# NikNazarov/TorchPIV

Measured on AMD Instinct MI355X. Metric: image-pairs/sec at 4 MP, wind=64 ov=32 2-pass CWS; % HBM roofline, higher is better.
Workload: dtype u32 exact sums + f64 / f32

## Files before the change

torchpiv_amd/csrc/xcorr_exact.hip:

```cpp
#include <hip/hip_runtime.h>
#include <stdint.h>
#include <stdlib.h>

#include "piv_kernels.h"
#include "xcorr_tile.hpp"

namespace tpiv {

namespace {

template <int W>
struct XGeo {
    static constexpr int NDW = W / 4;
    static constexpr int XP = 2 * NDW + 1;
    static constexpr int GROUP = W < 64 ? W : 64;
    static constexpr int WPW = 64 / GROUP;
    static constexpr int PARTS = W / GROUP;
    static constexpr int WAVES = W == 128 || W == 64 ? 2 : 4;
    static constexpr int WINS = WAVES * WPW / PARTS;
    static constexpr int KD = W * W;
    static constexpr bool COOP = W >= 32;
    static constexpr int P16 = W / 16;
    static constexpr int LW = GROUP * PARTS;
    static constexpr int AP = NDW + 4;
    static_assert(!COOP || (W * AP <= W * XP && (LW * P16) == W * P16), "the hand-over tile lives in the parked rows' memory");
};
constexpr int XCELLS = 5 + EXACT_MAX_SECOND + EXACT_MAX_MIN;

#if defined(__HIP_DEVICE_COMPILE__)
template <int OFF>
__device__ __forceinline__ uint32_t lds_rd32(unsigned addr) {
    uint32_t v;
    asm volatile("ds_read_b32 %0, %1 offset:%2" : "=v"(v) : "v"(addr), "n"(OFF) : "memory");
    return v;
}
__device__ __forceinline__ void lds_landed() { asm volatile("s_waitcnt lgkmcnt(0)" ::: "memory"); }
__device__ __forceinline__ void lds_tie(uint32_t& v) { asm volatile("" : "+v"(v)); }
#else
template <int OFF>
__host__ __device__ inline uint32_t lds_rd32(unsigned) { return 0u; }
__host__ __device__ inline void lds_landed() {}
__host__ __device__ inline void lds_tie(uint32_t&) {}
#endif
template <int N>
__device__ __forceinline__ void read_span(const uint32_t* src, uint32_t (&w)[N]) {
    const unsigned addr = (unsigned)(uintptr_t)src;
    static_for<0, N>([&](auto ic) TPIV_LAMBDA_INLINE { w[decltype(ic)::value] = lds_rd32<4 * decltype(ic)::value>(addr); });
    lds_landed();
    static_for<0, N>([&](auto ic) TPIV_LAMBDA_INLINE { lds_tie(w[decltype(ic)::value]); });
}

__device__ __forceinline__ void list_append(const PassParams& p, bool want, long long it) {
    const unsigned long long mk = __ballot(want);
    if (mk == 0ull) return;
    const int lane = (int)__builtin_amdgcn_mbcnt_hi(~0u, __builtin_amdgcn_mbcnt_lo(~0u, 0u));
    const int leader = (int)__builtin_ctzll(mk);
    unsigned base = 0u;
    if (lane == leader) base = atomicAdd(p.fb_count, (unsigned)__popcll(mk));
    base = (unsigned)__builtin_amdgcn_readlane((int)base, leader);
    if (want) p.fb_list[base + (unsigned)__popcll(mk & ((1ull << lane) - 1ull))] = (int)it;
}

__device__ __forceinline__ void decide_and_store(const PassParams& p, const uint4& rec, int r0, bool go, bool writer, bool have,
                                                 int m, unsigned S, unsigned sa, unsigned sb, double kd, double* out, long long it) {
    auto hi16 = [](unsigned v) TPIV_LAMBDA_INLINE { return (int)(short)(v >> 16); };
    auto umin = [](unsigned x, unsigned y) TPIV_LAMBDA_INLINE { return x < y ? x : y; };
    auto umax = [](unsigned x, unsigned y) TPIV_LAMBDA_INLINE { return x > y ? x : y; };
    auto uadd = [](unsigned x, unsigned y) TPIV_LAMBDA_INLINE { return x + y; };
    constexpr int S0 = 5, N0 = 5 + EXACT_MAX_SECOND;
    S = r0 < XCELLS ? S : 0u;
    const unsigned s_min = grp_reduce<16>((have && r0 >= N0 && r0 < XCELLS) ? S : 0xffffffffu, umin);
    const unsigned s_low = grp_reduce<16>((have && r0 < XCELLS) ? S : 0xffffffffu, umin);
    const unsigned s_top = grp_reduce<16>((have && r0 < N0) ? S : 0u, umax);
    const unsigned s_m = grp_reduce<16>(r0 == 0 ? S : 0u, umax);
    const unsigned s_second = grp_reduce<16>((have && r0 >= S0 && r0 < N0) ? S : 0u, umax);
    const unsigned n_second = grp_reduce<16>((have && r0 >= S0 && r0 < N0) ? 1u : 0u, uadd);
    const bool min_overflow = hi16(rec.w) == -2;
    const bool redo = s_top > s_m || s_low < s_min || s_min == 0xffffffffu || sa == 0u || sb == 0u ||
                      (min_overflow && s_min != 0u);
    list_append(p, go && redo && r0 == 0 && writer, it);
    const double scale = (kd * kd) / ((double)sa * (double)sb);
    const unsigned mine = r0 == 5 ? s_second : S;
    double v = __fma_rn((double)(mine - s_min), scale, 1e-7);
    v = (r0 == 5 && n_second == 0u) ? 0.0 : v;
    v = r0 == 6 ? (double)m : v;
    v = r0 == 7 ? 0.0 : v;
    if (go && !redo && r0 < 8 && writer) out[r0] = v;
}

template <int W>
__global__ __launch_bounds__(64 * XGeo<W>::WAVES) void xcorr_exact_refine_kernel(PassParams p) {
    using G = XGeo<W>;
    constexpr int NDW = G::NDW, XP = G::XP, KD = G::KD;
    __shared__ __attribute__((aligned(16))) uint32_t parked[G::WINS][W * XP];
    __shared__ unsigned joined[2][16];
    const int wave = __builtin_amdgcn_readfirstlane((int)(threadIdx.x >> 6));
    const int lane = (int)(threadIdx.x & 63);
    const int g = lane / G::GROUP, r0 = lane % G::GROUP;
    const int part = G::PARTS == 2 ? wave : 0;
    const int row = r0 + 64 * part;
    const int wslot = G::PARTS == 2 ? 0 : wave * G::WPW + g;
    uint32_t* const rows_b = parked[wslot];
    const int N = p.n_rows * p.n_cols;
    const long long total = (long long)p.batch * N;
    const int xcd = blockIdx.x & 7, slot = blockIdx.x >> 3;
    const long long chunk = (total + 7) / 8;
    const long long in_chunk = (long long)slot * G::WINS + wslot;
    const long long it_raw = (long long)xcd * chunk + in_chunk;
    const bool valid = in_chunk < chunk && it_raw < total;
    const long long it = valid ? it_raw : 0;

    const unsigned itu = (unsigned)it;
    const int pair = (int)(itu / (unsigned)N), win = (int)(itu - (unsigned)pair * (unsigned)N);
    const int st = p.ws - p.ov;
    const size_t off0 = (size_t)pair * p.H * p.W + (size_t)((win / p.n_cols) * st) * p.W + (size_t)(win % p.n_cols) * st;
    uint32_t a[NDW], b[NDW];
    uint32_t ca[G::COOP ? G::P16 : 1][4], cb[G::COOP ? G::P16 : 1][4];
    const int tw = r0 + 64 * part;
    if constexpr (G::COOP) {
#pragma unroll
        for (int k = 0; k < G::P16; ++k) {
            const int ci = tw + G::LW * k, j = ci / G::P16, pt = ci % G::P16;
            const size_t o_ = off0 + (size_t)j * p.W + 16 * pt;
            load_dwords<4>(p.A + o_, ca[k]);
            load_dwords<4>(p.B + o_, cb[k]);
        }
    } else {
        const size_t off = off0 + (size_t)row * p.W;
        load_dwords<NDW>(p.A + off, a);
        load_dwords<NDW>(p.B + off, b);
    }
    const uint4 rec = p.cand[it];
    auto lo16 = [](unsigned v) TPIV_LAMBDA_INLINE { return (int)(short)(v & 0xffffu); };
    auto hi16 = [](unsigned v) TPIV_LAMBDA_INLINE { return (int)(short)(v >> 16); };
    const int m = valid ? lo16(rec.x) : -3;
    double* const out = reinterpret_cast<double*>(p.peak_raw) + (size_t)it * 8;
    const bool writer = part == 0;
    list_append(p, m == -1 && r0 == 0 && writer, it);
    if (m == -2 && r0 < 8 && writer) out[r0] = r0 == 6 ? 0.0 : 1.0;
    const bool go = m >= 0;
    if (__ballot(go) == 0ull) return;
    bool nb_fast = false;
    if constexpr (G::COOP) {
        const bool regular = (m & (W - 1)) >= 1 && (m & (W - 1)) <= W - 2 && m + 1 < KD - 1 && m - 1 > 0 && m + W < KD - 1 &&
                             m - W > 0;
        nb_fast = __ballot(go && !regular) == 0ull;
    }

    int q = -1;
    if (go) {
        int left = m + 1, right = m - 1, top = m + W, bot = m - W;
        if (left >= KD - 1) left = m;
        if (right <= 0) right = m;
        if (top >= KD - 1) top = m;
        if (bot <= 0) bot = m;
        q = r0 == 0 ? m : q;
        q = r0 == 1 ? left : q;
        q = r0 == 2 ? right : q;
        q = r0 == 3 ? top : q;
        q = r0 == 4 ? bot : q;
        q = r0 == 5 ? hi16(rec.x) : q;
        q = r0 == 6 ? lo16(rec.y) : q;
        q = r0 == 7 ? hi16(rec.y) : q;
        q = r0 == 8 ? lo16(rec.z) : q;
        q = r0 == 9 ? hi16(rec.z) : q;
        q = r0 == 10 ? lo16(rec.w) : q;
        q = r0 == 11 ? hi16(rec.w) : q;
    }

    unsigned P[16];
#pragma unroll
    for (int k = 0; k < 16; ++k) P[k] = 0u;
    auto lds_sync = [&]() TPIV_LAMBDA_INLINE {
        if constexpr (G::PARTS == 2) __syncthreads();
        else wave_sync();
    };
    uint32_t au[NDW], ad[NDW];
    if constexpr (G::COOP) {
        uint4* const ta = reinterpret_cast<uint4*>(rows_b);
#pragma unroll
        for (int k = 0; k < G::P16; ++k) {
            const int ci = tw + G::LW * k, j = ci / G::P16, pt = ci % G::P16;
            ta[j * (G::AP / 4) + pt] = make_uint4(ca[k][0], ca[k][1], ca[k][2], ca[k][3]);
        }
        lds_sync();
#pragma unroll
        for (int k = 0; k < NDW / 4; ++k) {
            const uint4 t = ta[row * (G::AP / 4) + k];
            a[4 * k] = t.x, a[4 * k + 1] = t.y, a[4 * k + 2] = t.z, a[4 * k + 3] = t.w;
        }
        if (nb_fast) {
            const int ru = (row - 1) & (W - 1), rd = (row + 1) & (W - 1);
#pragma unroll
            for (int k = 0; k < NDW / 4; ++k) {
                const uint4 t = ta[ru * (G::AP / 4) + k], s = ta[rd * (G::AP / 4) + k];
                au[4 * k] = t.x, au[4 * k + 1] = t.y, au[4 * k + 2] = t.z, au[4 * k + 3] = t.w;
                ad[4 * k] = s.x, ad[4 * k + 1] = s.y, ad[4 * k + 2] = s.z, ad[4 * k + 3] = s.w;
            }
        }
        lds_sync();
#pragma unroll
        for (int k = 0; k < G::P16; ++k) {
            const int ci = tw + G::LW * k, j = ci / G::P16, pt = ci % G::P16;
#pragma unroll
            for (int c = 0; c < 4; ++c) {
                P[13] = __builtin_amdgcn_sad_u8(cb[k][c], 0u, P[13]);
                rows_b[j * XP + 4 * pt + c] = cb[k][c];
                rows_b[j * XP + NDW + 4 * pt + c] = cb[k][c];
            }
        }
#pragma unroll
        for (int i = 0; i < NDW; ++i) P[12] = __builtin_amdgcn_sad_u8(a[i], 0u, P[12]);
    } else {
#pragma unroll
        for (int i = 0; i < NDW; ++i) {
            P[12] = __builtin_amdgcn_sad_u8(a[i], 0u, P[12]);
            P[13] = __builtin_amdgcn_sad_u8(b[i], 0u, P[13]);
            rows_b[row * XP + i] = b[i];
            rows_b[row * XP + NDW + i] = b[i];
        }
    }
    lds_sync();

    if constexpr (G::COOP) {
        if (nb_fast) {
            const int mm = go ? m : KD / 2 + W / 2;
            const int dy = mm / W - W / 2, s = (mm % W - W / 2 - 1) & (W - 1);
            const int brow = (row + dy) & (W - 1);
            uint32_t w[NDW + 2];
            read_span<NDW + 2>(rows_b + brow * XP + (s >> 2), w);
            w[NDW + 1] = s == W - 1 ? w[1] : w[NDW + 1];
            uint32_t u[NDW + 1];
#pragma unroll
            for (int i = 0; i <= NDW; ++i) u[i] = __builtin_amdgcn_alignbyte(w[i + 1], w[i], (unsigned)(s & 3));
            unsigned s_m = 0u, s_l = 0u, s_r = 0u, s_t = 0u, s_b = 0u;
#pragma unroll
            for (int i = 0; i < NDW; ++i) {
                const uint32_t c = __builtin_amdgcn_alignbyte(u[i + 1], u[i], 1u);
                s_r = __builtin_amdgcn_udot4(a[i], u[i], s_r, false);
                s_m = __builtin_amdgcn_udot4(a[i], c, s_m, false);
                s_l = __builtin_amdgcn_udot4(a[i], __builtin_amdgcn_alignbyte(u[i + 1], u[i], 2u), s_l, false);
                s_t = __builtin_amdgcn_udot4(au[i], c, s_t, false);
                s_b = __builtin_amdgcn_udot4(ad[i], c, s_b, false);
            }
            P[0] = go ? s_m : 0u, P[1] = go ? s_l : 0u, P[2] = go ? s_r : 0u, P[3] = go ? s_t : 0u, P[4] = go ? s_b : 0u;
        }
    }
    static_for<0, XCELLS>([&](auto cc) TPIV_LAMBDA_INLINE {
        constexpr int c = decltype(cc)::value;
        if (c < 5 && nb_fast) return;
        int qc = __builtin_amdgcn_readlane(q, c);
        bool any = qc >= 0;
        static_for<1, G::WPW>([&](auto wc) TPIV_LAMBDA_INLINE {
            constexpr int k = decltype(wc)::value;
            const int qk = __builtin_amdgcn_readlane(q, k * G::GROUP + c);
            any = any || qk >= 0;
            qc = g == k ? qk : qc;
        });
        if (any) {
            const bool on = qc >= 0;
            const int qq = on ? qc : 0;
            const int dy = qq / W - W / 2, dx = qq % W - W / 2;
            const int brow = (row + dy) & (W - 1), bx = dx & (W - 1);
            const uint32_t* src = rows_b + brow * XP + (bx >> 2);
            const unsigned sh = (unsigned)(bx & 3);
            uint32_t w[NDW + 1];
            read_span<NDW + 1>(src, w);
            unsigned acc = 0;
#pragma unroll
            for (int i = 0; i < NDW; ++i) acc = __builtin_amdgcn_udot4(a[i], __builtin_amdgcn_alignbyte(w[i + 1], w[i], sh), acc, false);
            P[c] = on ? acc : 0u;
        }
    });
    unsigned T[4];
    {
        const bool odd = lane & 1, hi = lane & 2;
        unsigned Q[8];
#pragma unroll
        for (int j = 0; j < 8; ++j) {
            const unsigned keep = odd ? P[2 * j + 1] : P[2 * j], send = odd ? P[2 * j] : P[2 * j + 1];
            Q[j] = keep + (unsigned)dpp_i<DPP_XOR1>((int)send);
        }
#pragma unroll
        for (int j = 0; j < 4; ++j) {
            const unsigned keep = hi ? Q[2 * j + 1] : Q[2 * j], send = hi ? Q[2 * j] : Q[2 * j + 1];
            unsigned t = keep + (unsigned)dpp_i<DPP_XOR2>((int)send);
            t += (unsigned)dpp_i<0x128>((int)t);
            t += (unsigned)dpp_i<0x124>((int)t);
            if constexpr (G::GROUP >= 32) {
                auto r = __builtin_amdgcn_permlane16_swap(t, t, false, false);
                t = r[0] + r[1];
            }
            if constexpr (G::GROUP >= 64) {
                auto r = __builtin_amdgcn_permlane32_swap(t, t, false, false);
                t = r[0] + r[1];
            }
            T[j] = t;
        }
    }
    unsigned S = r0 < 4 ? T[0] : (r0 < 8 ? T[1] : (r0 < 12 ? T[2] : T[3]));
    if constexpr (G::PARTS == 2) {
        if (lane < 16) joined[wave][lane] = S;
        __syncthreads();
        S = lane < 16 ? joined[0][lane] + joined[1][lane] : 0u;
        T[3] = S;
    }
    unsigned sa, sb;
    {
        const unsigned t3 = (r0 & 12) == 12 ? T[3] : 0u;
        unsigned rowsum = t3;
        rowsum += (unsigned)dpp_i<0x128>((int)rowsum);
        rowsum += (unsigned)dpp_i<0x124>((int)rowsum);
        sa = (unsigned)dpp_i<0x00>((int)rowsum);
        sb = (unsigned)dpp_i<0x55>((int)rowsum);
    }
    S = r0 < XCELLS ? S : 0u;

    decide_and_store(p, rec, r0, go, writer, q >= 0, m, S, sa, sb, (double)KD, out, it);
}

template <int W>
struct SGeo {
    static constexpr int NDW = W / 4, XP = 2 * NDW + 1, STRIP = (W * XP) | 1, KD = W * W;
};
template <int W>
struct SBlock {
    static constexpr int SW = W == 8 ? 4 : 1;
};
template <int W>
__global__ __launch_bounds__(64 * SBlock<W>::SW) void xcorr_exact_refine_small_kernel(PassParams p) {
    using G = SGeo<W>;
    constexpr int NDW = G::NDW, XP = G::XP, KD = G::KD, SW = SBlock<W>::SW, NT = 64 * SW;
    __shared__ uint32_t strips[NT * G::STRIP];
    __shared__ unsigned blk_n, blk_base;
    const int lane = (int)threadIdx.x;
    uint32_t* const mine = strips + lane * G::STRIP;
    if (SW > 1 && lane == 0) blk_n = 0u;
    const int N = p.n_rows * p.n_cols;
    const long long total = (long long)p.batch * N;
    const int xcd = blockIdx.x & 7, slot = blockIdx.x >> 3;
    const long long chunk = (total + 7) / 8;
    const long long in_chunk = (long long)slot * NT + lane;
    const long long it_raw = (long long)xcd * chunk + in_chunk;
    const bool valid = in_chunk < chunk && it_raw < total;
    const long long it = valid ? it_raw : 0;
    const unsigned itu = (unsigned)it;
    const int pair = (int)(itu / (unsigned)N), win = (int)(itu - (unsigned)pair * (unsigned)N);
    const int st = p.ws - p.ov;
    const size_t off = (size_t)pair * p.H * p.W + (size_t)((win / p.n_cols) * st) * p.W + (size_t)(win % p.n_cols) * st;
    const uint4 rec = p.cand[it];
    uint32_t a[W][NDW];
    unsigned sa = 0u, sb = 0u;
#pragma unroll
    for (int y = 0; y < W; ++y) {
        uint32_t b[NDW];
        load_dwords<NDW>(p.A + off + (size_t)y * p.W, a[y]);
        load_dwords<NDW>(p.B + off + (size_t)y * p.W, b);
#pragma unroll
        for (int i = 0; i < NDW; ++i) {
            sa = __builtin_amdgcn_sad_u8(a[y][i], 0u, sa);
            sb = __builtin_amdgcn_sad_u8(b[i], 0u, sb);
            mine[y * XP + i] = b[i];
            mine[y * XP + NDW + i] = b[i];
        }
    }
    auto lo16 = [](unsigned v) TPIV_LAMBDA_INLINE { return (int)(short)(v & 0xffffu); };
    auto hi16 = [](unsigned v) TPIV_LAMBDA_INLINE { return (int)(short)(v >> 16); };
    const int m = valid ? lo16(rec.x) : -3;
    double* const out = reinterpret_cast<double*>(p.peak_raw) + (size_t)it * 8;
    if (m == -2) {
#pragma unroll
        for (int r = 0; r < 8; ++r) out[r] = r == 6 ? 0.0 : 1.0;
    }
    const bool go = m >= 0;
    bool redo = false;
    if (__ballot(go) != 0ull) {
    int q[XCELLS];
    {
        int left = m + 1, right = m - 1, top = m + W, bot = m - W;
        if (left >= KD - 1) left = m;
        if (right <= 0) right = m;
        if (top >= KD - 1) top = m;
        if (bot <= 0) bot = m;
        q[0] = m, q[1] = left, q[2] = right, q[3] = top, q[4] = bot;
        q[5] = hi16(rec.x), q[6] = lo16(rec.y), q[7] = hi16(rec.y);
        q[8] = lo16(rec.z), q[9] = hi16(rec.z), q[10] = lo16(rec.w), q[11] = hi16(rec.w);
    }
    wave_sync();
    unsigned S[XCELLS];
    static_for<0, XCELLS>([&](auto cc) TPIV_LAMBDA_INLINE {
        constexpr int c = decltype(cc)::value;
        const bool on = go && q[c] >= 0;
        unsigned acc = 0u;
        if (__ballot(on) != 0ull) {
            const int qq = on ? q[c] : 0;
            const int dy = qq / W - W / 2, bx = (qq % W - W / 2) & (W - 1);
            const unsigned sh = (unsigned)(bx & 3);
            const uint32_t* const src = mine + (bx >> 2);
#pragma unroll
            for (int y = 0; y < W; ++y) {
                const uint32_t* rowp = src + ((y + dy) & (W - 1)) * XP;
                uint32_t w[NDW + 1];
#pragma unroll
                for (int i = 0; i <= NDW; ++i) w[i] = rowp[i];
#pragma unroll
                for (int i = 0; i < NDW; ++i) acc = __builtin_amdgcn_udot4(a[y][i], __builtin_amdgcn_alignbyte(w[i + 1], w[i], sh), acc, false);
            }
        }
        S[c] = on ? acc : 0u;
    });
    constexpr int S0 = 5, N0 = 5 + EXACT_MAX_SECOND;
    unsigned s_min = 0xffffffffu, s_low = 0xffffffffu, s_top = 0u, s_second = 0u, n_second = 0u;
#pragma unroll
    for (int c = 0; c < XCELLS; ++c) {
        const bool have = q[c] >= 0;
        if (c >= N0) s_min = (have && S[c] < s_min) ? S[c] : s_min;
        s_low = (have && S[c] < s_low) ? S[c] : s_low;
        if (c < N0) s_top = (have && S[c] > s_top) ? S[c] : s_top;
        if (c >= S0 && c < N0) {
            s_second = (have && S[c] > s_second) ? S[c] : s_second;
            n_second += have ? 1u : 0u;
        }
    }
    const unsigned s_m = S[0];
    const bool min_overflow = hi16(rec.w) == -2;
    redo = s_top > s_m || s_low < s_min || s_min == 0xffffffffu || sa == 0u || sb == 0u || (min_overflow && s_min != 0u);
    if (go && !redo) {
        const double scale = ((double)KD * (double)KD) / ((double)sa * (double)sb);
#pragma unroll
        for (int r = 0; r < 5; ++r) out[r] = __fma_rn((double)(S[r] - s_min), scale, 1e-7);
        out[5] = n_second == 0u ? 0.0 : __fma_rn((double)(s_second - s_min), scale, 1e-7);
        out[6] = (double)m;
        out[7] = 0.0;
    }
    }
    const bool want = m == -1 || (go && redo);
    if constexpr (SW == 1) {
        list_append(p, want, it);
    } else {
        const unsigned long long mk = __ballot(want);
        const int wl = lane & 63;
        unsigned wbase = 0u;
        __syncthreads();
        if (mk != 0ull && wl == 0) wbase = atomicAdd(&blk_n, (unsigned)__popcll(mk));
        wbase = (unsigned)__builtin_amdgcn_readfirstlane((int)wbase);
        __syncthreads();
        if (lane == 0 && blk_n != 0u) blk_base = atomicAdd(p.fb_count, blk_n);
        __syncthreads();
        if (want) p.fb_list[blk_base + wbase + (unsigned)__popcll(mk & ((1ull << wl) - 1ull))] = (int)it;
    }
}

template <int G>
__global__ __launch_bounds__(64) void xcorr_exact_refine_any_kernel(PassParams p, int ndw, int xp) {
    extern __shared__ uint32_t any_smem[];
    constexpr int LPW = 64 / G, SL = LPW / 16;
    const int W = p.ws, KD = W * W;
    const int lane = (int)threadIdx.x;
    const int g = lane / LPW, c = lane & 15, k = (lane % LPW) >> 4;
    const int N = p.n_rows * p.n_cols;
    const long long total = (long long)p.batch * N;
    const int xcd = blockIdx.x & 7, slot = blockIdx.x >> 3;
    const long long chunk = (total + 7) / 8;
    const int st = p.ws - p.ov;
    const bool dwords = (W & 3) == 0;
    const float rcp_ndw = 1.0f / (float)ndw;

    unsigned sa_w[G], sb_w[G];
    long long it_w[G];
    bool valid_w[G];
    static_for<0, G>([&](auto gc) TPIV_LAMBDA_INLINE {
        constexpr int gi = decltype(gc)::value;
        const long long in_chunk = (long long)slot * G + gi;
        const long long it_raw = (long long)xcd * chunk + in_chunk;
        valid_w[gi] = in_chunk < chunk && it_raw < total;
        it_w[gi] = valid_w[gi] ? it_raw : 0;
        const unsigned itu = (unsigned)it_w[gi];
        const int pair = (int)(itu / (unsigned)N), win = (int)(itu - (unsigned)pair * (unsigned)N);
        const size_t off = (size_t)pair * p.H * p.W + (size_t)((win / p.n_cols) * st) * p.W + (size_t)(win % p.n_cols) * st;
        const uint8_t* __restrict__ A0 = p.A + off;
        const uint8_t* __restrict__ B0 = p.B + off;
        uint32_t* const ag = any_smem + gi * W * ndw;
        uint32_t* const bg = any_smem + G * W * ndw + gi * W * xp;
        uint8_t* const bgb = reinterpret_cast<uint8_t*>(bg);
        unsigned pa = 0u, pb = 0u;
        for (int idx = lane; idx < W * ndw; idx += 64) {
            const int row = (int)(((float)idx + 0.5f) * rcp_ndw), i = idx - row * ndw;
            const uint8_t* ra = A0 + (size_t)row * p.W + 4 * i;
            const uint8_t* rb = B0 + (size_t)row * p.W + 4 * i;
            uint32_t da = 0u, db = 0u;
            const int nb = W - 4 * i < 4 ? W - 4 * i : 4;
            if (nb == 4) {
                __builtin_memcpy(&da, ra, 4);
                __builtin_memcpy(&db, rb, 4);
            } else {
                for (int t = 0; t < nb; ++t) {
                    da |= (uint32_t)ra[t] << (8 * t);
                    db |= (uint32_t)rb[t] << (8 * t);
                }
            }
            ag[row * ndw + i] = da;
            pa = __builtin_amdgcn_sad_u8(da, 0u, pa);
            pb = __builtin_amdgcn_sad_u8(db, 0u, pb);
            if (dwords) {
                bg[row * xp + i] = db;
                bg[row * xp + ndw + i] = db;
            } else {
                for (int t = 0; t < nb; ++t) {
                    const uint8_t v = (uint8_t)(db >> (8 * t));
                    bgb[row * xp * 4 + 4 * i + t] = v;
                    bgb[row * xp * 4 + W + 4 * i + t] = v;
                }
            }
        }
        auto uadd = [](unsigned x, unsigned y) TPIV_LAMBDA_INLINE { return x + y; };
        sa_w[gi] = grp_reduce<64>(pa, uadd);
        sb_w[gi] = grp_reduce<64>(pb, uadd);
    });
    wave_sync();

    long long it = it_w[0];
    bool valid = valid_w[0];
    unsigned sa = sa_w[0], sb = sb_w[0];
    static_for<1, G>([&](auto gc) TPIV_LAMBDA_INLINE {
        constexpr int gi = decltype(gc)::value;
        it = g == gi ? it_w[gi] : it;
        valid = g == gi ? valid_w[gi] : valid;
        sa = g == gi ? sa_w[gi] : sa;
        sb = g == gi ? sb_w[gi] : sb;
    });
    const uint4 rec = p.cand[it];
    auto lo16 = [](unsigned v) TPIV_LAMBDA_INLINE { return (int)(short)(v & 0xffffu); };
    auto hi16 = [](unsigned v) TPIV_LAMBDA_INLINE { return (int)(short)(v >> 16); };
    const int m = valid ? lo16(rec.x) : -3;
    double* const out = reinterpret_cast<double*>(p.peak_raw) + (size_t)it * 8;
    const bool writer = k == 0;
    list_append(p, m == -1 && c == 0 && writer, it);
    if (m == -2 && c < 8 && writer) out[c] = c == 6 ? 0.0 : 1.0;
    const bool go = m >= 0;
    if (__ballot(go) == 0ull) return;
    int q = -1;
    if (go) {
        int left = m + 1, right = m - 1, top = m + W, bot = m - W;
        if (left >= KD - 1) left = m;
        if (right <= 0) right = m;
        if (top >= KD - 1) top = m;
        if (bot <= 0) bot = m;
        q = c == 0 ? m : q;
        q = c == 1 ? left : q;
        q = c == 2 ? right : q;
        q = c == 3 ? top : q;
        q = c == 4 ? bot : q;
        q = c == 5 ? hi16(rec.x) : q;
        q = c == 6 ? lo16(rec.y) : q;
        q = c == 7 ? hi16(rec.y) : q;
        q = c == 8 ? lo16(rec.z) : q;
        q = c == 9 ? hi16(rec.z) : q;
        q = c == 10 ? lo16(rec.w) : q;
        q = c == 11 ? hi16(rec.w) : q;
    }
    unsigned S = 0u;
    {
        const bool on = q >= 0;
        const int qq = on ? q : 0;
        const int qy = qq / W, qx = qq - qy * W;
        int dy = qy - W / 2, bx = qx - W / 2;
        bx += bx < 0 ? W : 0;
        const unsigned sh = (unsigned)(bx & 3);
        const uint32_t* const ag = any_smem + g * W * ndw;
        const uint32_t* const bg = any_smem + G * W * ndw + g * W * xp + (bx >> 2);
        for (int y = k; y < W; y += SL) {
            int by = y + dy;
            by += by < 0 ? W : 0;
            by -= by >= W ? W : 0;
            const uint32_t* ar = ag + y * ndw;
            const uint32_t* br = bg + by * xp;
            uint32_t prev = br[0];
            for (int i = 0; i < ndw; ++i) {
                const uint32_t nxt = br[i + 1];
                S = __builtin_amdgcn_udot4(ar[i], __builtin_amdgcn_alignbyte(nxt, prev, sh), S, false);
                prev = nxt;
            }
        }
        S = on ? S : 0u;
    }
    if constexpr (SL == 4) {
        auto r = __builtin_amdgcn_permlane16_swap(S, S, false, false);
        S = r[0] + r[1];
        auto r2 = __builtin_amdgcn_permlane32_swap(S, S, false, false);
        S = r2[0] + r2[1];
    }
    decide_and_store(p, rec, c, go, writer, q >= 0, m, S, sa, sb, (double)KD, out, it);
}

}

template <int W>
static hipError_t launch_refine(const PassParams& p, hipStream_t stream) {
    using G = XGeo<W>;
    const long long total = (long long)p.batch * p.n_rows * p.n_cols;
    const long long chunk = (total + 7) / 8;
    const long long slots = (chunk + G::WINS - 1) / G::WINS;
    hipLaunchKernelGGL((xcorr_exact_refine_kernel<W>), dim3((unsigned)(slots * 8)), dim3(64 * G::WAVES), 0, stream, p);
    return hipGetLastError();
}

template <int W>
static hipError_t launch_refine_small(const PassParams& p, hipStream_t stream) {
    const long long total = (long long)p.batch * p.n_rows * p.n_cols;
    const long long chunk = (total + 7) / 8;
    constexpr int NT = 64 * SBlock<W>::SW;
    const long long slots = (chunk + NT - 1) / NT;
    hipLaunchKernelGGL((xcorr_exact_refine_small_kernel<W>), dim3((unsigned)(slots * 8)), dim3(NT), 0, stream, p);
    return hipGetLastError();
}

template <int G>
static hipError_t launch_refine_any(const PassParams& p, hipStream_t stream) {
    const int W = p.ws, ndw = (W + 3) / 4;
    const int xp = ((2 * W + 6 + 3) / 4) | 1;
    const long long total = (long long)p.batch * p.n_rows * p.n_cols;
    const long long chunk = (total + 7) / 8;
    const long long slots = (chunk + G - 1) / G;
    const size_t smem = (size_t)G * W * (ndw + xp) * sizeof(uint32_t);
    if (smem > 64 * 1024) return hipErrorInvalidValue;
    hipLaunchKernelGGL((xcorr_exact_refine_any_kernel<G>), dim3((unsigned)(slots * 8)), dim3(64), smem, stream, p, ndw, xp);
    return hipGetLastError();
}

bool exact_refine_size(int ws) { return ws >= 8 && ws <= 128 && (ws & 1) == 0; }

hipError_t launch_exact_refine(const PassParams& p, int n_cu, hipStream_t stream) {
    const long long total = (long long)p.batch * p.n_rows * p.n_cols;
    if (total <= 0 || total >= (1ll << 31) || p.cand == nullptr || p.fb_list == nullptr || p.fb_count == nullptr ||
        !exact_refine_size(p.ws))
        return hipErrorInvalidValue;
    static const bool small_on = [] { const char* e = getenv("TPIV_REFINE_SMALL"); return !(e && e[0] == '0'); }();
    switch (p.ws) {
        case 8:
            if (small_on) return launch_refine_small<8>(p, stream);
            return launch_refine_any<4>(p, stream);
        case 16: return small_on ? launch_refine_small<16>(p, stream) : launch_refine<16>(p, stream);
        case 32: return launch_refine<32>(p, stream);
        case 64: return launch_refine<64>(p, stream);
        case 128: return launch_refine<128>(p, stream);
        default: return p.ws <= 32 ? launch_refine_any<4>(p, stream) : launch_refine_any<1>(p, stream);
    }
}

}
```

Measured before the change: 18160.

## Use 128-bit LDS reads and padded quad-aligned rows for 64-wide exact refine

Result: no change. 18240, median of 2 (+0.4%).

```diff
diff --git a/torchpiv_amd/csrc/xcorr_exact.hip b/torchpiv_amd/csrc/xcorr_exact.hip
--- a/torchpiv_amd/csrc/xcorr_exact.hip
+++ b/torchpiv_amd/csrc/xcorr_exact.hip
@@ -12,7 +12,8 @@
 template <int W>
 struct XGeo {
     static constexpr int NDW = W / 4;
-    static constexpr int XP = 2 * NDW + 1;
+    static constexpr bool Q16 = W == 64;
+    static constexpr int XP = Q16 ? 2 * NDW + 4 : 2 * NDW + 1;
     static constexpr int GROUP = W < 64 ? W : 64;
     static constexpr int WPW = 64 / GROUP;
     static constexpr int PARTS = W / GROUP;
@@ -27,6 +28,19 @@
 };
 constexpr int XCELLS = 5 + EXACT_MAX_SECOND + EXACT_MAX_MIN;
 
+template <int W>
+__device__ __forceinline__ void chunk_of(int t, int k, int& j, int& pt) {
+    using G = XGeo<W>;
+    if constexpr (G::Q16) {
+        pt = t & 3;
+        j = 4 * ((t >> 2) & 3) + (t >> 4) + 16 * k;
+    } else {
+        const int ci = t + G::LW * k;
+        j = ci / G::P16, pt = ci % G::P16;
+    }
+}
+
+typedef uint32_t u32x4 __attribute__((ext_vector_type(4)));
 #if defined(__HIP_DEVICE_COMPILE__)
 template <int OFF>
 __device__ __forceinline__ uint32_t lds_rd32(unsigned addr) {
@@ -34,13 +48,23 @@
     asm volatile("ds_read_b32 %0, %1 offset:%2" : "=v"(v) : "v"(addr), "n"(OFF) : "memory");
     return v;
 }
+template <int OFF>
+__device__ __forceinline__ u32x4 lds_rd128(unsigned addr) {
+    u32x4 v;
+    asm volatile("ds_read_b128 %0, %1 offset:%2" : "=v"(v) : "v"(addr), "n"(OFF) : "memory");
+    return v;
+}
 __device__ __forceinline__ void lds_landed() { asm volatile("s_waitcnt lgkmcnt(0)" ::: "memory"); }
 __device__ __forceinline__ void lds_tie(uint32_t& v) { asm volatile("" : "+v"(v)); }
+__device__ __forceinline__ void lds_tie(u32x4& v) { asm volatile("" : "+v"(v)); }
 #else
 template <int OFF>
 __host__ __device__ inline uint32_t lds_rd32(unsigned) { return 0u; }
+template <int OFF>
+__host__ __device__ inline u32x4 lds_rd128(unsigned) { return u32x4{0u, 0u, 0u, 0u}; }
 __host__ __device__ inline void lds_landed() {}
 __host__ __device__ inline void lds_tie(uint32_t&) {}
+__host__ __device__ inline void lds_tie(u32x4&) {}
 #endif
 template <int N>
 __device__ __forceinline__ void read_span(const uint32_t* src, uint32_t (&w)[N]) {
@@ -48,6 +72,18 @@
     static_for<0, N>([&](auto ic) TPIV_LAMBDA_INLINE { w[decltype(ic)::value] = lds_rd32<4 * decltype(ic)::value>(addr); });
     lds_landed();
     static_for<0, N>([&](auto ic) TPIV_LAMBDA_INLINE { lds_tie(w[decltype(ic)::value]); });
+}
+template <int NQ>
+__device__ __forceinline__ void read_quads(const uint32_t* src, uint32_t (&w)[4 * NQ]) {
+    const unsigned addr = (unsigned)(uintptr_t)src;
+    u32x4 t[NQ];
+    static_for<0, NQ>([&](auto ic) TPIV_LAMBDA_INLINE { t[decltype(ic)::value] = lds_rd128<16 * decltype(ic)::value>(addr); });
+    lds_landed();
+    static_for<0, NQ>([&](auto ic) TPIV_LAMBDA_INLINE {
+        constexpr int i = decltype(ic)::value;
+        lds_tie(t[i]);
+        w[4 * i] = t[i].x, w[4 * i + 1] = t[i].y, w[4 * i + 2] = t[i].z, w[4 * i + 3] = t[i].w;
+    });
 }
 
 __device__ __forceinline__ void list_append(const PassParams& p, bool want, long long it) {
@@ -110,17 +146,18 @@
     const bool valid = in_chunk < chunk && it_raw < total;
     const long long it = valid ? it_raw : 0;
 
-    const unsigned itu = (unsigned)it;
-    const int pair = (int)(itu / (unsigned)N), win = (int)(itu - (unsigned)pair * (unsigned)N);
+    const int pair = fast_div((int)it, p.groups_magic, p.groups_shift), win = (int)it - pair * N;
+    const int wrow = fast_div(win, p.ncols_magic, p.ncols_shift), wcol = win - wrow * p.n_cols;
     const int st = p.ws - p.ov;
-    const size_t off0 = (size_t)pair * p.H * p.W + (size_t)((win / p.n_cols) * st) * p.W + (size_t)(win % p.n_cols) * st;
+    const size_t off0 = (size_t)pair * p.H * p.W + (size_t)(wrow * st) * p.W + (size_t)wcol * st;
     uint32_t a[NDW], b[NDW];
     uint32_t ca[G::COOP ? G::P16 : 1][4], cb[G::COOP ? G::P16 : 1][4];
     const int tw = r0 + 64 * part;
     if constexpr (G::COOP) {
 #pragma unroll
         for (int k = 0; k < G::P16; ++k) {
-            const int ci = tw + G::LW * k, j = ci / G::P16, pt = ci % G::P16;
+            int j, pt;
+            chunk_of<W>(tw, k, j, pt);
             const size_t o_ = off0 + (size_t)j * p.W + 16 * pt;
             load_dwords<4>(p.A + o_, ca[k]);
             load_dwords<4>(p.B + o_, cb[k]);
@@ -180,7 +217,8 @@
         uint4* const ta = reinterpret_cast<uint4*>(rows_b);
 #pragma unroll
         for (int k = 0; k < G::P16; ++k) {
-            const int ci = tw + G::LW * k, j = ci / G::P16, pt = ci % G::P16;
+            int j, pt;
+            chunk_of<W>(tw, k, j, pt);
             ta[j * (G::AP / 4) + pt] = make_uint4(ca[k][0], ca[k][1], ca[k][2], ca[k][3]);
         }
         lds_sync();
@@ -201,12 +239,19 @@
         lds_sync();
 #pragma unroll
         for (int k = 0; k < G::P16; ++k) {
-            const int ci = tw + G::LW * k, j = ci / G::P16, pt = ci % G::P16;
-#pragma unroll
-            for (int c = 0; c < 4; ++c) {
-                P[13] = __builtin_amdgcn_sad_u8(cb[k][c], 0u, P[13]);
-                rows_b[j * XP + 4 * pt + c] = cb[k][c];
-                rows_b[j * XP + NDW + 4 * pt + c] = cb[k][c];
+            int j, pt;
+            chunk_of<W>(tw, k, j, pt);
+#pragma unroll
+            for (int c = 0; c < 4; ++c) P[13] = __builtin_amdgcn_sad_u8(cb[k][c], 0u, P[13]);
+            if constexpr (G::Q16) {
+                uint4* const tb = reinterpret_cast<uint4*>(rows_b) + j * (XP / 4) + pt;
+                tb[0] = tb[NDW / 4] = make_uint4(cb[k][0], cb[k][1], cb[k][2], cb[k][3]);
+            } else {
+#pragma unroll
+                for (int c = 0; c < 4; ++c) {
+                    rows_b[j * XP + 4 * pt + c] = cb[k][c];
+                    rows_b[j * XP + NDW + 4 * pt + c] = cb[k][c];
+                }
             }
         }
 #pragma unroll
@@ -227,12 +272,26 @@
             const int mm = go ? m : KD / 2 + W / 2;
             const int dy = mm / W - W / 2, s = (mm % W - W / 2 - 1) & (W - 1);
             const int brow = (row + dy) & (W - 1);
-            uint32_t w[NDW + 2];
-            read_span<NDW + 2>(rows_b + brow * XP + (s >> 2), w);
-            w[NDW + 1] = s == W - 1 ? w[1] : w[NDW + 1];
             uint32_t u[NDW + 1];
-#pragma unroll
-            for (int i = 0; i <= NDW; ++i) u[i] = __builtin_amdgcn_alignbyte(w[i + 1], w[i], (unsigned)(s & 3));
+            if constexpr (G::Q16) {
+                const int su = __builtin_amdgcn_readfirstlane(s);
+                uint32_t w[24];
+                read_quads<6>(rows_b + brow * XP + ((s >> 2) & ~3), w);
+                static_for<0, 4>([&](auto oc) TPIV_LAMBDA_INLINE {
+                    constexpr int O = decltype(oc)::value;
+                    if (((su >> 2) & 3) == O) {
+                        if constexpr (O == 3) w[20] = su == W - 1 ? w[4] : w[20];
+#pragma unroll
+                        for (int i = 0; i <= NDW; ++i) u[i] = __builtin_amdgcn_alignbyte(w[O + i + 1], w[O + i], (unsigned)(su & 3));
+                    }
+                });
+            } else {
+                uint32_t w[NDW + 2];
+                read_span<NDW + 2>(rows_b + brow * XP + (s >> 2), w);
+                w[NDW + 1] = s == W - 1 ? w[1] : w[NDW + 1];
+#pragma unroll
+                for (int i = 0; i <= NDW; ++i) u[i] = __builtin_amdgcn_alignbyte(w[i + 1], w[i], (unsigned)(s & 3));
+            }
             unsigned s_m = 0u, s_l = 0u, s_r = 0u, s_t = 0u, s_b = 0u;
 #pragma unroll
             for (int i = 0; i < NDW; ++i) {
@@ -262,13 +321,25 @@
             const int qq = on ? qc : 0;
             const int dy = qq / W - W / 2, dx = qq % W - W / 2;
             const int brow = (row + dy) & (W - 1), bx = dx & (W - 1);
-            const uint32_t* src = rows_b + brow * XP + (bx >> 2);
             const unsigned sh = (unsigned)(bx & 3);
-            uint32_t w[NDW + 1];
-            read_span<NDW + 1>(src, w);
             unsigned acc = 0;
-#pragma unroll
-            for (int i = 0; i < NDW; ++i) acc = __builtin_amdgcn_udot4(a[i], __builtin_amdgcn_alignbyte(w[i + 1], w[i], sh), acc, false);
+            if constexpr (G::Q16) {
+                uint32_t w[20];
+                read_quads<5>(rows_b + brow * XP + ((bx >> 2) & ~3), w);
+                static_for<0, 4>([&](auto oc) TPIV_LAMBDA_INLINE {
+                    constexpr int O = decltype(oc)::value;
+                    if (((bx >> 2) & 3) == O) {
+#pragma unroll
+                        for (int i = 0; i < NDW; ++i)
+                            acc = __builtin_amdgcn_udot4(a[i], __builtin_amdgcn_alignbyte(w[O + i + 1], w[O + i], sh), acc, false);
+                    }
+                });
+            } else {
+                uint32_t w[NDW + 1];
+                read_span<NDW + 1>(rows_b + brow * XP + (bx >> 2), w);
+#pragma unroll
+                for (int i = 0; i < NDW; ++i) acc = __builtin_amdgcn_udot4(a[i], __builtin_amdgcn_alignbyte(w[i + 1], w[i], sh), acc, false);
+            }
             P[c] = on ? acc : 0u;
         }
     });
@@ -601,7 +672,10 @@
     const long long total = (long long)p.batch * p.n_rows * p.n_cols;
     const long long chunk = (total + 7) / 8;
     const long long slots = (chunk + G::WINS - 1) / G::WINS;
-    hipLaunchKernelGGL((xcorr_exact_refine_kernel<W>), dim3((unsigned)(slots * 8)), dim3(64 * G::WAVES), 0, stream, p);
+    PassParams q = p;
+    fast_div_setup((unsigned)(p.n_rows * p.n_cols), q.groups_magic, q.groups_shift);
+    fast_div_setup((unsigned)p.n_cols, q.ncols_magic, q.ncols_shift);
+    hipLaunchKernelGGL((xcorr_exact_refine_kernel<W>), dim3((unsigned)(slots * 8)), dim3(64 * G::WAVES), 0, stream, q);
     return hipGetLastError();
 }
 
```
